# gonewest818/raytrace-clj

Hardware: NVIDIA B200
Metric: samples_per_sec (higher is better)
Workload: dtype f32

## Files before the change

### raytrace_clj_b200/csrc/rt_kernels.cuh

```cuda
#pragma once

#include "rt_device.cuh"

namespace rt {

#define RT_FOR_R _Pragma("unroll") for (int r = 0; r < R; ++r)

struct PathBounce {
    float o[3];
    float time;
    float d[3];
    int hit_id;
    double t;
};

struct RenderParams {
    DevScene sc;
    DevCamera cam;
    int nx, ny;
    int sample_begin, sample_count;
    int row_offset, row_stride, rows_in_shard;
    int max_depth;
    uint2 key;
    float* sum;
// ... 440 lines not shown
    }
}

template <int R, int BLOCK>
struct PairSink {
    unsigned idx0;
    unsigned n;
    unsigned n_g, p0;
    __device__ __forceinline__ unsigned entry(unsigned v) const { return v < n_g ? v : p0 + (v - n_g); }
    unsigned long long live;
    uint2* pairs;
    unsigned pair_cap;
    unsigned long long* best_key;
    WaveState* st;

    __device__ __forceinline__ void flush(const uint32_t* list, unsigned long long nz, int count, int kbase) {
        nz &= live;
        if (!__any_sync(0xffffffffu, nz != 0ull)) return;
        const unsigned lane = threadIdx.x & 31u;
        unsigned np = 0;
        for (unsigned long long z = nz; z; z &= z - 1ull) {
            const int i = __ffsll((long long)z) - 1;
            np += __popc(~Culler<R, BLOCK>::word(list, i & 15, i >> 4));
        }
        unsigned incl = np;
#pragma unroll
        for (int d = 1; d < 32; d <<= 1) {
            unsigned v = __shfl_up_sync(0xffffffffu, incl, d);
            if ((int)lane >= d) incl += v;
        }
        const unsigned total = __shfl_sync(0xffffffffu, incl, 31);
        unsigned base = 0;
        if (lane == 0) base = atomicAdd(&st->npairs, total);
        base = __shfl_sync(0xffffffffu, base, 0);
        const bool fits = base + total <= pair_cap;
        unsigned w = base + incl - np;
        SurvivorIter<R, BLOCK> it;
        it.begin(nz, count);
        int r, k;
        while (it.next(list, r, k)) {
            const unsigned v = idx0 + 32u * (unsigned)r;
            if (fits) {
                pairs[w] = make_uint2(entry(v), (unsigned)(kbase + k));
            } else {
                if (w < pair_cap) pairs[w] = make_uint2(PAIR_NULL, 0u);
                if (v < n) best_key[entry(v)] = BEST_KEY_OVERFLOW;
            }
            ++w;
        }
    }
};

constexpr unsigned ITEM_NONE = 0xffffffffu;
constexpr unsigned ITEM_STOP = 0xfffffffeu;
struct Scope {
    unsigned bid, nblk;
};
__device__ __forceinline__ Scope grid_scope() { return Scope{blockIdx.x, gridDim.x}; }
template <int R, int BLOCK, bool COMMON>
__device__ __forceinline__ unsigned wf_cull_batches(const WaveParams& W, Scope sc_, int cur, unsigned e0, unsigned e1, unsigned n_g,
                                                    unsigned p0, unsigned long long gen0, int parts, unsigned item0, unsigned claimed,
                                                    int& budget, float4* s_cull, uint32_t* s_list) {
    if (claimed == ITEM_STOP) return ITEM_STOP;
    const RenderParams& P = W.base;
    const unsigned lane = threadIdx.x & 31u, warp = threadIdx.x >> 5, warps = BLOCK / 32;
    const unsigned n_batches = (e1 - e0 + 32 * R - 1) / (32 * R);
    const unsigned n_items = n_batches * (unsigned)parts;
    Culler<R, BLOCK, COMMON> K;
    K.cox = P.cam.origin.x; K.coy = P.cam.origin.y; K.coz = P.cam.origin.z;
    PairSink<R, BLOCK> sink;
    sink.n = e1;
    sink.n_g = n_g;
    sink.p0 = p0;
    sink.pairs = W.pairs;
    sink.pair_cap = W.pair_cap;
    sink.best_key = W.best_key;
    sink.st = W.st;
    unsigned item = sc_.bid * warps + warp;
    const unsigned uniform_end = (n_items + warps - 1) / warps * warps;
    for (;;) {
        if (P.preloaded) {
            if (claimed != ITEM_NONE) {
                item = claimed;
                claimed = ITEM_NONE;
            } else {
                unsigned b = 0;
                if (lane == 0) b = atomicAdd(&W.st->batch, 1u);
                item = __shfl_sync(0xffffffffu, b, 0);
            }
            if (item >= item0 + n_items) return item;
            item -= item0;
        } else {
            if (item - warp >= uniform_end) break;
        }
        const unsigned batch = item / (unsigned)parts, part = item - batch * (unsigned)parts;
        sink.idx0 = e0 + batch * (32 * R) + lane;
        sink.live = 0ull;
        RT_FOR_R {
            const unsigned v = sink.idx0 + 32 * r;
            if (v < e1 && batch < n_batches) {
                float4* qc = cur ? W.queue[1] : W.queue[0];
                float4 a, b;
                if (v >= n_g) {
                    float4 c;
                    float4* q = qc + 3 * (size_t)(p0 + (v - n_g));
                    make_path(P, gen0 + (v - n_g), a, b, c);
                    if (part == 0) { q[0] = a; q[1] = b; q[2] = c; }
                } else {
                    a = qc[3 * (size_t)v];
                    b = qc[3 * (size_t)v + 1];
                }
                K.set_ray(r, a.x, a.y, a.z, b.x, b.y, b.z);
                sink.live |= 0xffffull << (16 * r);
            } else {
                K.kill(r);
            }
        }
        if (parts > 1) K.run_slice(P.sc, s_cull, s_list, sink, (int)part, parts);
        else           K.run(P.sc, s_cull, P.cull_cap, P.preloaded != 0, s_list, sink);
        item += sc_.nblk * warps;
        if (P.preloaded && budget > 0 && --budget == 0) return ITEM_STOP;
    }
    return ITEM_NONE;
}

template <int R, int BLOCK>
__device__ __forceinline__ void wf_cull_body(const WaveParams& W, Scope sc_, int cur, unsigned n_g, unsigned n_p, unsigned long long gen_base,
                                             float4* s_cull, float4* s_cullc, uint32_t* s_list) {
    const RenderParams& P = W.base;
    const unsigned n = n_g + n_p, p0 = (unsigned)W.capacity - n_p;
    if (sc_.bid == 0 && threadIdx.x == 0) atomicAdd(&P.counters[DC_RAYS], (unsigned long long)n);
    const unsigned grid_warps = W.resident_warps > 0 ? (unsigned)W.resident_warps : sc_.nblk * (BLOCK / 32);
    int budget = W.claims_per_warp;
    const unsigned n_c = P.common_origin ? n_p : 0u, n_v = n - n_c;
    const unsigned long long genC = gen_base - p0;
    if (R > 1 && !P.preloaded) {
        if (n_c) wf_cull_batches<R, BLOCK, true>(W, sc_, cur, p0, p0 + n_c, 0u, 0u, genC + 0u, 1, 0u, ITEM_NONE, budget, s_cull, s_list);
        if (n_v) wf_cull_batches<R, BLOCK, false>(W, sc_, cur, 0u, n_v, n_g, p0, gen_base, 1, 0u, ITEM_NONE, budget, s_cull, s_list);
    } else if (R > 1 && n >= grid_warps * 64u) {
        const unsigned tail = grid_warps * 64u, per = 32u * R;
        const unsigned g_rest0 = min(n_v, tail), p_rest0 = min(n_c, tail - g_rest0);
        const unsigned g_bulk = (n_v - g_rest0) / per * per, p_bulk = (n_c - p_rest0) / per * per;
        unsigned items = 0;
        unsigned next = wf_cull_batches<R, BLOCK, true>(W, sc_, cur, p0, p0 + p_bulk, 0u, 0u, genC, 1, items, ITEM_NONE, budget, s_cullc, s_list);
        items += p_bulk / per;
        next = wf_cull_batches<R, BLOCK, false>(W, sc_, cur, 0u, g_bulk, n_g, p0, gen_base, 1, items, next, budget, s_cull, s_list);
        items += g_bulk / per;
        next = wf_cull_batches<1, BLOCK, true>(W, sc_, cur, p0 + p_bulk, p0 + n_c, 0u, 0u, genC, 1, items, next, budget, s_cullc, s_list);
        items += (n_c - p_bulk + 31u) / 32u;
        wf_cull_batches<1, BLOCK, false>(W, sc_, cur, g_bulk, n_v, n_g, p0, gen_base, 1, items, next, budget, s_cull, s_list);
    } else {
        const unsigned b1 = (n + 31) / 32;
        int parts = 1;
        if (P.preloaded)
            while (parts < 16 && b1 * (unsigned)parts * 2u <= grid_warps) parts *= 2;
        unsigned next = ITEM_NONE, items = 0;
        if (n_c) {
            next = wf_cull_batches<1, BLOCK, true>(W, sc_, cur, p0, p0 + n_c, 0u, 0u, genC, parts, 0u, ITEM_NONE, budget, P.preloaded ? s_cullc : s_cull, s_list);
            items = (n_c + 31u) / 32u * (unsigned)parts;
        }
        if (n_v) wf_cull_batches<1, BLOCK, false>(W, sc_, cur, 0u, n_v, n_g, p0, gen_base, parts, items, next, budget, s_cull, s_list);
    }
}

template <int R, int BLOCK, int MINB>
__global__ void __launch_bounds__(BLOCK, MINB) wf_cull(const __grid_constant__ WaveParams W) {
    TraceScope trace(W.trace);
    const RenderParams& P = W.base;
    extern __shared__ float4 smem_f4[];
    float4* s_cull = smem_f4;
    uint32_t* s_list = reinterpret_cast<uint32_t*>(smem_f4 + P.cull_cap);
    float4* s_cullc = reinterpret_cast<float4*>(s_list + Culler<R, BLOCK>::LIST_WORDS * BLOCK);
    if (W.st->mode != MODE_RUN) return;
    const unsigned n_g = W.st->cnt[W.cur][0], n_p = W.st->cnt[W.cur][1];
    if (n_g + n_p == 0) return;
    const unsigned long long gen_base = W.st->gen_base[W.cur];
    if (P.preloaded) {
        preload_scene(P.sc, s_cull, BLOCK);
        if (n_p && P.common_origin)
            for (int i = threadIdx.x; i < P.sc.n_cull; i += BLOCK)
                s_cullc[i] = Culler<R, BLOCK, true>::common_record(s_cull[i], P.cam.origin.x, P.cam.origin.y, P.cam.origin.z);
    }
    __syncthreads();
    wf_cull_body<R, BLOCK>(W, grid_scope(), W.cur, n_g, n_p, gen_base, s_cull, s_cullc, s_list);
}

#include "rt_cull_tc.cuh"

__device__ __forceinline__ unsigned wf_cand_region(const WaveParams& W, unsigned total_warps) {
    return ((W.pair_cap + total_warps * 32u - 1u) / (total_warps * 32u)) * 32u;
}

template <bool GEN>
__device__ __forceinline__ void wf_refine_body(const WaveParams& W, const DevScene* scp, Scope sc_, int cur) {
    const RenderParams& P = W.base;
    const unsigned npairs = min(W.st->npairs, W.pair_cap);
    const unsigned lane = threadIdx.x & 31u;
    if (sc_.bid == 0 && threadIdx.x == 0) {
        W.st->batch = 0;
        W.st->cnt[cur ^ 1][0] = 0;
        W.st->cnt[cur ^ 1][1] = 0;
        atomicAdd(&P.counters[DC_CANDIDATES], (unsigned long long)(npairs - min(npairs, W.st->pad)));
        W.st->pad = 0;
    }
    const unsigned total_warps = sc_.nblk * (blockDim.x >> 5);
    const unsigned warp_id = sc_.bid * (blockDim.x >> 5) + (threadIdx.x >> 5);
    const size_t region = (size_t)warp_id * wf_cand_region(W, total_warps);
    unsigned cnt = 0;
    const unsigned stride = sc_.nblk * blockDim.x;
    const unsigned i_first = sc_.bid * blockDim.x + threadIdx.x;
    uint2 pr_next = i_first < npairs ? W.pairs[i_first] : make_uint2(PAIR_NULL, 0u);
    for (unsigned i0 = i_first - lane; i0 < npairs; i0 += stride) {
        const uint2 pr = pr_next;
        const unsigned i_next = i0 + lane + stride;
        pr_next = i_next < npairs ? W.pairs[i_next] : make_uint2(PAIR_NULL, 0u);
        bool cand = false;
        double t = CUDART_INF;
        if (pr.x != PAIR_NULL) {
            const float4* qc = cur ? W.queue[1] : W.queue[0];
            const float4 a = qc[3 * (size_t)pr.x], b = qc[3 * (size_t)pr.x + 1];
            const unsigned long long seen = __ldcg(&W.best_t[pr.x]);
            if (!GEN) {
                t = refine_candidate(P.sc.ex_c0r, P.sc.ex_c1, P.sc.ex_t0t1, P.sc.flags, (int)pr.y, a.x, a.y, a.z, b.x, b.y, b.z,
                                     a.w, 0.001, (double)FLT_MAX);
            } else {
                uint32_t pixq = 0, smpq = 0, bq = 0;
                if (__ldg(&P.sc.prim_type[pr.y]) == PRIM_MEDIUM) {
                    const uint32_t sd = __float_as_uint(qc[3 * (size_t)pr.x + 2].w);
                    pixq = rng_pixel(P, __float_as_uint(b.w));
                    smpq = sd >> 8;
                    bq = (uint32_t)(P.max_depth - (int)(sd & 255u) + 1);
                }
                t = refine_leaf<true>(scp, (int)pr.y, a.x, a.y, a.z, b.x, b.y, b.z, a.w, 0.001, (double)FLT_MAX, true, P.key, pixq, smpq, bq);
            }
            const unsigned long long tb = (unsigned long long)__double_as_longlong(t);
            if (t < CUDART_INF && tb <= seen) {
                atomicMin(&W.best_t[pr.x], tb);
                cand = true;
            }
        }
        const unsigned m = __ballot_sync(0xffffffffu, cand);
        if (cand) {
            const size_t slot = region + cnt + __popc(m & ((1u << lane) - 1u));
            W.cands[slot] = pr;
            W.cand_t[slot] = t;
        }
        cnt += __popc(m);
    }
    if (lane == 0) W.cand_count[warp_id] = cnt;
}
template <bool GEN>
__global__ void __launch_bounds__(256) wf_refine(const __grid_constant__ WaveParams W) {
    if (W.st->mode != MODE_RUN) return;
    TraceScope trace(W.trace);
    wf_refine_body<GEN>(W, &W.base.sc, grid_scope(), W.cur);
}

__device__ __forceinline__ void wf_tiebreak_body(const WaveParams& W, Scope sc_) {
    const RenderParams& P = W.base;
    const unsigned lane = threadIdx.x & 31u;
    const unsigned total_warps = sc_.nblk * (blockDim.x >> 5);
    const unsigned warp_id = sc_.bid * (blockDim.x >> 5) + (threadIdx.x >> 5);
    const size_t region = (size_t)warp_id * wf_cand_region(W, total_warps);
    const unsigned cnt = W.cand_count[warp_id];
    for (unsigned j = lane; j < cnt; j += 32) {
        const uint2 pr = W.cands[region + j];
        if ((unsigned long long)__double_as_longlong(W.cand_t[region + j]) == W.best_t[pr.x])
            atomicMin(&W.best_key[pr.x], (((unsigned long long)__ldg(&P.sc.tie_hi[pr.y])) << 32) | pr.y);
    }
}
__global__ void __launch_bounds__(256) wf_tiebreak(const __grid_constant__ WaveParams W) {
    if (W.st->mode != MODE_RUN) return;
    TraceScope trace(W.trace);
    wf_tiebreak_body(W, grid_scope());
}

template <bool GEN>
__device__ __noinline__ void exact_closest_hit(const DevScene* sc, float ox, float oy, float oz, float dx, float dy, float dz,
                                               float tm, uint2 key, uint32_t pixel, uint32_t sample, uint32_t bounce, double* out_t,
                                               int* out_k) {
    double best = CUDART_INF;
    int bk = -1;
    unsigned btie = 0xffffffffu;
    for (int k = 0; k < sc->n; ++k) {
        double t = refine_leaf<GEN>(sc, k, ox, oy, oz, dx, dy, dz, tm, 0.001, (double)FLT_MAX, true, key, pixel, sample, bounce);
        if (t < CUDART_INF) {
            unsigned tie = __ldg(&sc->tie_hi[k]);
            if (t < best || (t == best && tie < btie)) { best = t; bk = k; btie = tie; }
        }
    }
    *out_t = best;
    *out_k = bk;
}

template <bool GEN>
__device__ __forceinline__ unsigned wf_shade_body(const WaveParams& W, const DevScene* scp, Scope sc_, int cur, unsigned* s_ctr) {
    const RenderParams& P = W.base;
    const unsigned n_g = W.st->cnt[cur][0], n_p = W.st->cnt[cur][1], n = n_g + n_p;
    const unsigned lane = threadIdx.x & 31u;
    const float4* qc = cur ? W.queue[1] : W.queue[0];
    float4* qn = cur ? W.queue[0] : W.queue[1];
    if (sc_.bid == 0 && threadIdx.x == 0) W.st->npairs = 0;
    unsigned n_direct = 0;
    const unsigned stride = sc_.nblk * blockDim.x;
    for (unsigned idx0 = sc_.bid * blockDim.x + threadIdx.x - lane; idx0 < n; idx0 += stride) {
        const bool have = idx0 + lane < n;
        const unsigned idx = wf_entry(idx0 + lane, n_g, n_p, (unsigned)W.capacity);
        bool cont = false;
        float4 a, b, c;
        if (have) {
            a = qc[3 * (size_t)idx]; b = qc[3 * (size_t)idx + 1]; c = qc[3 * (size_t)idx + 2];
            unsigned long long key = W.best_key[idx];
            const uint32_t slot = __float_as_uint(b.w), sd = __float_as_uint(c.w);
            const uint32_t pix = rng_pixel(P, slot);
            const uint32_t smp = sd >> 8;
            const int depth = (int)(sd & 255u);
            const uint32_t bounce = (uint32_t)(P.max_depth - depth + 1);
            int k = (int)(unsigned)key;
            double td = __longlong_as_double((long long)W.best_t[idx]);
            W.best_key[idx] = BEST_KEY_MISS;
            W.best_t[idx] = BEST_T_INIT;
            if (key == BEST_KEY_OVERFLOW) {
                exact_closest_hit<GEN>(scp, a.x, a.y, a.z, b.x, b.y, b.z, a.w, P.key, pix, smp, bounce, &td, &k);
                key = k < 0 ? BEST_KEY_MISS : 1ull;
            } else {
                for (int kd = P.sc.n_list; kd < P.sc.n; ++kd) {
                    ++n_direct;
                    const double t = refine_leaf<GEN>(scp, kd, a.x, a.y, a.z, b.x, b.y, b.z, a.w, 0.001, (double)FLT_MAX, true, P.key, pix,
                                                      smp, bounce);
                    const unsigned long long kk = (((unsigned long long)__ldg(&P.sc.tie_hi[kd])) << 32) | (unsigned)kd;
                    if (t < td || (t < CUDART_INF && t == td && kk < key)) {
                        td = t;
                        key = kk;
                        k = kd;
                    }
                }
            }
            const bool hit = key != BEST_KEY_MISS;
            if (P.path_pixel) path_log_ray(P, slot, (int)bounce - 1, a, b, hit ? k : -1, hit ? td : CUDART_INF);
            if (!hit) {
                atomicAdd(&s_ctr[DC_TERM_MISS], 1u);
                if (P.path_pixel) path_log_end(P, slot, (int)bounce, TERM_MISS);
            } else {
                float3 o = f3(a.x, a.y, a.z), d = f3(b.x, b.y, b.z);
                float3 att, em;
                int reason = TERM_NONE;
                float tmv = a.w;
                ScatterRng rng{P.key, pix, smp, bounce, nullptr, nullptr};
                cont = shade_hit<GEN>(P.sc, scp, k, (float)td, o, d, tmv, depth > 0, rng, att, em, reason);
                if (em.x != 0.f || em.y != 0.f || em.z != 0.f) {
                    float* dst = P.sum + (size_t)slot * 3;
                    atomicAdd(dst + 0, c.x * em.x);
                    atomicAdd(dst + 1, c.y * em.y);
                    atomicAdd(dst + 2, c.z * em.z);
                }
                if (cont) {
                    a = make_float4(o.x, o.y, o.z, tmv);
                    b = make_float4(d.x, d.y, d.z, b.w);
                    c = make_float4(c.x * att.x, c.y * att.y, c.z * att.z, __uint_as_float((smp << 8) | (uint32_t)(depth - 1)));
                } else {
                    atomicAdd(&s_ctr[reason == TERM_LIGHT ? DC_TERM_LIGHT
                                     : reason == TERM_ABSORB ? DC_TERM_ABSORB : DC_TERM_DEPTH], 1u);
                    if (P.path_pixel) path_log_end(P, slot, (int)bounce, reason);
                }
            }
        }
        const unsigned mc = __ballot_sync(0xffffffffu, cont);
        if (mc) {
            unsigned base = 0u;
            if (lane == 0) base = atomicAdd(&W.st->cnt[cur ^ 1][0], (unsigned)__popc(mc));
            base = __shfl_sync(0xffffffffu, base, 0);
            if (cont) {
                float4* q = qn + 3 * (size_t)(base + __popc(mc & ((1u << lane) - 1u)));
                q[0] = a; q[1] = b; q[2] = c;
            }
        }
    }
    if (n_direct) atomicAdd(&s_ctr[DC_DIRECT], n_direct);
    return 0u;
}

template <bool GEN>
__global__ void __launch_bounds__(256, GEN ? 1 : 0) wf_shade(const __grid_constant__ WaveParams W) {
    if (W.st->mode != MODE_RUN) return;
    TraceScope trace(W.trace);
    const RenderParams& P = W.base;
    __shared__ unsigned s_ctr[DC_COUNT];
    if (threadIdx.x < DC_COUNT) s_ctr[threadIdx.x] = 0;
    __syncthreads();
    wf_shade_body<GEN>(W, &W.base.sc, grid_scope(), W.cur, s_ctr);
    __syncthreads();
    if (threadIdx.x < DC_COUNT && s_ctr[threadIdx.x]) atomicAdd(&P.counters[threadIdx.x], (unsigned long long)s_ctr[threadIdx.x]);
    if (threadIdx.x == 0) {
        __threadfence();
        if (atomicAdd(&W.st->done, 1u) == gridDim.x - 1) {
            __threadfence();
            W.st->done = 0;
            const unsigned n_cont = *(volatile unsigned*)&W.st->cnt[W.cur ^ 1][0];
            const unsigned want = (unsigned)W.capacity - n_cont;
            unsigned n_fresh = 0;
            unsigned long long base = 0ull;
            if (!W.st->exhausted && want) {
                base = atomicAdd(P.work_counter, (unsigned long long)want);
                if (base < P.total_work) n_fresh = (unsigned)min((unsigned long long)want, P.total_work - base);
                if (base + want >= P.total_work) W.st->exhausted = 1u;
            }
            W.st->cnt[W.cur ^ 1][1] = n_fresh;
            W.st->gen_base[W.cur ^ 1] = base;
            if (n_fresh) atomicAdd(&P.counters[DC_SAMPLES], (unsigned long long)n_fresh);
            if (n_cont + n_fresh == 0) W.st->mode = MODE_DONE;
            __threadfence();
            publish_status(W, n_cont + n_fresh, n_fresh, W.st->exhausted, W.st->mode, W.iter);
        }
    }
}

struct TraceParamsB {
    DevScene sc;
    int n;
    const float* origins;
    const float* dirs;
    const float* times;
    double tmin, tmax;
    double* out_t;
    int* out_id;
    unsigned long long* stats;
};

struct BvhHit {
    double t;
    int k;
    unsigned tie;
    unsigned n_leaf, n_node;
};
template <bool GEN>
__device__ __forceinline__ BvhHit bvh_closest(const DevScene* sc, float ox, float oy, float oz, float dx, float dy, float dz, float time,
                                              double tmin, double tmax, bool has_ctx, uint2 key, uint32_t pixel, uint32_t sample,
                                              uint32_t bounce) {
    BvhHit H{CUDART_INF, -1, 0xffffffffu, 0u, 0u};
    const float ix = 1.0f / dx, iy = 1.0f / dy, iz = 1.0f / dz;
    const float e = 2.4e-7f * fmaxf(fmaxf(fabsf(ox), fabsf(oy)), fabsf(oz));
    const float tlo = (float)tmin * (1.0f - 1e-6f);
    float thi = tmax >= (double)FLT_MAX ? FLT_MAX : __double2float_ru(tmax);
    int stack[48];
    int sp = 0, node = 0;
    for (;;) {
        if (node >= 0) {
            const float4 A = __ldg(&sc->bvh[4 * node]), B = __ldg(&sc->bvh[4 * node + 1]), C = __ldg(&sc->bvh[4 * node + 2]);
            const int4 D = __ldg(reinterpret_cast<const int4*>(&sc->bvh[4 * node + 3]));
            H.n_node += 2;
            float a0 = ((A.x - e) - ox) * ix, a1 = ((A.w + e) - ox) * ix, b0 = ((A.y - e) - oy) * iy, b1 = ((B.x + e) - oy) * iy,
                  c0 = ((A.z - e) - oz) * iz, c1 = ((B.y + e) - oz) * iz;
            float ln = fmaxf(fmaxf(fminf(a0, a1), fminf(b0, b1)), fmaxf(fminf(c0, c1), tlo));
            float lf = fminf(fminf(fmaxf(a0, a1), fmaxf(b0, b1)), fminf(fmaxf(c0, c1), thi));
            a0 = ((B.z - e) - ox) * ix; a1 = ((C.y + e) - ox) * ix; b0 = ((B.w - e) - oy) * iy; b1 = ((C.z + e) - oy) * iy;
            c0 = ((C.x - e) - oz) * iz; c1 = ((C.w + e) - oz) * iz;
            float rn = fmaxf(fmaxf(fminf(a0, a1), fminf(b0, b1)), fmaxf(fminf(c0, c1), tlo));
            float rf = fminf(fminf(fmaxf(a0, a1), fmaxf(b0, b1)), fminf(fmaxf(c0, c1), thi));
            const bool hl = ln <= lf * 1.0000005f + 1e-30f, hr = rn <= rf * 1.0000005f + 1e-30f;
            if (hl && hr) {
                const bool left_first = ln <= rn;
                stack[sp++] = left_first ? D.y : D.x;
                node = left_first ? D.x : D.y;
                continue;
            }
            if (hl) { node = D.x; continue; }
            if (hr) { node = D.y; continue; }
        } else {
            const int k = ~node;
            H.n_leaf++;
            const double t = refine_leaf<GEN>(sc, k, ox, oy, oz, dx, dy, dz, time, tmin, tmax, has_ctx, key, pixel, sample, bounce);
            if (t < CUDART_INF) {
                const unsigned tie = __ldg(&sc->tie_hi[k]);
                if (t < H.t || (t == H.t && tie < H.tie)) {
                    H.t = t; H.k = k; H.tie = tie;
                    thi = fminf(thi, __double2float_ru(t));
                }
            }
        }
        if (sp == 0) break;
        node = stack[--sp];
    }
    return H;
}

template <bool GEN>
__global__ void __launch_bounds__(128, GEN ? 1 : 0) wf_bvh(const __grid_constant__ WaveParams W) {
    if (W.st->mode != MODE_RUN) return;
    TraceScope trace(W.trace);
    const RenderParams& P = W.base;
    __shared__ unsigned s_ctr[DC_COUNT];
    if (threadIdx.x < DC_COUNT) s_ctr[threadIdx.x] = 0;
    __syncthreads();
    const int cur = W.cur;
    const unsigned n_g = W.st->cnt[cur][0], n_p = W.st->cnt[cur][1], n = n_g + n_p, p0 = (unsigned)W.capacity - n_p;
    const unsigned long long gen_base = W.st->gen_base[cur];
    float4* qc = cur ? W.queue[1] : W.queue[0];
    unsigned n_leaf = 0, n_node = 0;
    for (unsigned v = blockIdx.x * blockDim.x + threadIdx.x; v < n; v += gridDim.x * blockDim.x) {
        float4 a, b, c;
        unsigned idx;
        if (v >= n_g) {
            idx = p0 + (v - n_g);
            make_path(P, gen_base + (v - n_g), a, b, c);
            float4* q = qc + 3 * (size_t)idx;
            q[0] = a; q[1] = b; q[2] = c;
        } else {
            idx = v;
            a = qc[3 * (size_t)idx]; b = qc[3 * (size_t)idx + 1]; c = qc[3 * (size_t)idx + 2];
        }
        const uint32_t sd = __float_as_uint(c.w);
        const BvhHit H = bvh_closest<GEN>(&W.base.sc, a.x, a.y, a.z, b.x, b.y, b.z, a.w, 0.001, (double)FLT_MAX, true, P.key,
                                          rng_pixel(P, __float_as_uint(b.w)), sd >> 8, (uint32_t)(P.max_depth - (int)(sd & 255u) + 1));
        n_leaf += H.n_leaf; n_node += H.n_node;
        if (H.k >= 0) {
            W.best_t[idx] = (unsigned long long)__double_as_longlong(H.t);
            W.best_key[idx] = ((unsigned long long)H.tie << 32) | (unsigned)H.k;
        }
    }
    atomicAdd(&s_ctr[DC_CANDIDATES], n_leaf);
    atomicAdd(&s_ctr[DC_BVH_NODES], n_node);
    __syncthreads();
    if (threadIdx.x < DC_COUNT && s_ctr[threadIdx.x]) atomicAdd(&P.counters[threadIdx.x], (unsigned long long)s_ctr[threadIdx.x]);
    if (blockIdx.x == 0 && threadIdx.x == 0) {
        atomicAdd(&P.counters[DC_RAYS], (unsigned long long)n);
        W.st->batch = 0;
        W.st->npairs = 0;
        W.st->cnt[cur ^ 1][0] = 0;
        W.st->cnt[cur ^ 1][1] = 0;
    }
}

template <bool GEN>
__global__ void __launch_bounds__(128) trace_bvh_kernel(const __grid_constant__ TraceParamsB P) {
    const int idx = blockIdx.x * blockDim.x + threadIdx.x;
    if (idx >= P.n) return;
    const float ox = P.origins[3 * idx], oy = P.origins[3 * idx + 1], oz = P.origins[3 * idx + 2];
    const float dx = P.dirs[3 * idx], dy = P.dirs[3 * idx + 1], dz = P.dirs[3 * idx + 2];
    const float tm = P.times ? P.times[idx] : 0.f;
    BvhHit H = bvh_closest<GEN>(&P.sc, ox, oy, oz, dx, dy, dz, tm, P.tmin, P.tmax, false, make_uint2(0u, 0u), 0u, 0u, 0u);
    for (int k = P.sc.n_list; k < P.sc.n; ++k) {
        const double t = refine_leaf<GEN>(&P.sc, k, ox, oy, oz, dx, dy, dz, tm, P.tmin, P.tmax, false, make_uint2(0u, 0u), 0u, 0u, 0u);
        const unsigned tie = __ldg(&P.sc.tie_hi[k]);
        if (t < H.t || (t < CUDART_INF && t == H.t && tie < H.tie)) { H.t = t; H.k = k; H.tie = tie; }
    }
    P.out_t[idx] = H.t;
    P.out_id[idx] = H.k >= 0 ? __ldg(&P.sc.orig_id[H.k]) : -1;
    if (P.stats) {
        atomicAdd(&P.stats[0], (unsigned long long)H.n_leaf);
        atomicAdd(&P.stats[1], (unsigned long long)H.n_node);
    }
}

template <bool GEN>
__device__ __forceinline__ void wf_solo_paths(const WaveParams& W, const DevScene* scp, const float4* qc, unsigned n, unsigned* claim,
                                              const float4* s_cull, unsigned* s_ctr) {
    const RenderParams& P = W.base;
    const unsigned lane = threadIdx.x & 31u;
    const unsigned lpp = W.tail_lpp;
    const unsigned sub = lane & (lpp - 1u), lead = lane & ~(lpp - 1u);
    bool active = false;
    float4 a = make_float4(0.f, 0.f, 0.f, 0.f), b = a, c = a;
    uint32_t slot = 0u, pix = 0u;
    unsigned n_rays = 0, n_cand = 0, n_direct = 0;
    for (;;) {
        unsigned i = 0xffffffffu;
        if (!active && sub == 0u) i = atomicAdd(claim, 1u);
        i = __shfl_sync(0xffffffffu, i, (int)lead);
        if (!active && i < n) {
            a = qc[3 * (size_t)i]; b = qc[3 * (size_t)i + 1]; c = qc[3 * (size_t)i + 2];
            slot = __float_as_uint(b.w);
            pix = rng_pixel(P, slot);
            active = true;
        }
        if (!__any_sync(0xffffffffu, active)) break;
        const uint32_t sd = __float_as_uint(c.w), smp = sd >> 8;
        const int depth = (int)(sd & 255u);
        const uint32_t bounce = (uint32_t)(P.max_depth - depth + 1);
        Culler<1, 32, false> K;
        K.set_ray(0, a.x, a.y, a.z, b.x, b.y, b.z);
        if (active && sub == 0u) ++n_rays;
        unsigned long long bt = BEST_T_INIT, bkey = BEST_KEY_MISS;
        for (int base = 0; base < P.sc.n; base += 64 * (int)lpp) {
            unsigned long long mask = 0ull;
            if (active) {
                const int jn = min(64, (P.sc.n - base + (int)lpp - 1) / (int)lpp);
#pragma unroll 4
                for (int j = 0; j < jn; ++j) {
                    const int s = base + (int)lpp * j + (int)sub;
                    bool pass = s < P.sc.n;
                    if (s < P.sc.n_list) {
                        const float4 S = P.preloaded ? s_cull[s] : __ldg(&P.sc.cull_a[s]);
                        pass = (int)K.key_bits(S, 0) >= 0;
                    }
                    mask |= (unsigned long long)(pass ? 1u : 0u) << j;
                }
            }
            while (__any_sync(0xffffffffu, mask != 0ull)) {
                if (mask) {
                    const int s = base + (int)lpp * (__ffsll((long long)mask) - 1) + (int)sub;
                    mask &= mask - 1ull;
                    if (s < P.sc.n_list) ++n_cand; else ++n_direct;
                    const double t = refine_leaf<GEN>(scp, s, a.x, a.y, a.z, b.x, b.y, b.z, a.w, 0.001, (double)FLT_MAX, true, P.key, pix, smp,
                                                      bounce);
                    const unsigned long long tb = (unsigned long long)__double_as_longlong(t);
                    const unsigned long long kk = (((unsigned long long)__ldg(&P.sc.tie_hi[s])) << 32) | (unsigned)s;
                    if (t < CUDART_INF && (tb < bt || (tb == bt && kk < bkey))) { bt = tb; bkey = kk; }
                }
            }
        }
        for (unsigned dlt = lpp >> 1; dlt; dlt >>= 1) {
            const unsigned long long ot = __shfl_xor_sync(0xffffffffu, bt, (int)dlt), ok = __shfl_xor_sync(0xffffffffu, bkey, (int)dlt);
            if (ot < bt || (ot == bt && ok < bkey)) { bt = ot; bkey = ok; }
        }
        if (active) {
            const bool hit = bkey != BEST_KEY_MISS;
            const int k = (int)(unsigned)bkey;
            const double td = __longlong_as_double((long long)bt);
            if (P.path_pixel && sub == 0u) path_log_ray(P, slot, (int)bounce - 1, a, b, hit ? k : -1, hit ? td : CUDART_INF);
            int reason = TERM_MISS;
            bool cont = false;
            if (hit) {
                float3 o = f3(a.x, a.y, a.z), d = f3(b.x, b.y, b.z);
                float3 att, em;
                float tmv = a.w;
                ScatterRng rng{P.key, pix, smp, bounce, nullptr, nullptr};
                reason = TERM_NONE;
                cont = shade_hit<GEN>(P.sc, scp, k, (float)td, o, d, tmv, depth > 0, rng, att, em, reason);
                if (sub == 0u && (em.x != 0.f || em.y != 0.f || em.z != 0.f)) {
                    float* dst = P.sum + (size_t)slot * 3;
                    atomicAdd(dst + 0, c.x * em.x);
                    atomicAdd(dst + 1, c.y * em.y);
                    atomicAdd(dst + 2, c.z * em.z);
                }
                if (cont) {
                    a = make_float4(o.x, o.y, o.z, tmv);
                    b = make_float4(d.x, d.y, d.z, b.w);
                    c = make_float4(c.x * att.x, c.y * att.y, c.z * att.z, __uint_as_float((smp << 8) | (uint32_t)(depth - 1)));
                }
            }
            if (!cont) {
                if (sub == 0u) {
                    atomicAdd(&s_ctr[reason == TERM_MISS ? DC_TERM_MISS : reason == TERM_LIGHT ? DC_TERM_LIGHT
                                     : reason == TERM_ABSORB ? DC_TERM_ABSORB : DC_TERM_DEPTH], 1u);
                    if (P.path_pixel) path_log_end(P, slot, (int)bounce, reason);
                }
                active = false;
            }
        }
    }
    if (n_rays) atomicAdd(&s_ctr[DC_RAYS], n_rays);
    if (n_cand) atomicAdd(&s_ctr[DC_CANDIDATES], n_cand);
    if (n_direct) atomicAdd(&s_ctr[DC_DIRECT], n_direct);
}

constexpr int kPairsPerEntry = 8;
template <int BLOCK, bool GEN, int TR>
__global__ void __launch_bounds__(BLOCK, GEN ? 1 : 2) wf_tail(const __grid_constant__ WaveParams W) {
    const RenderParams& P = W.base;
    extern __shared__ float4 smem_f4[];
    float4* s_cull = smem_f4;
    uint32_t* s_list = reinterpret_cast<uint32_t*>(smem_f4 + P.cull_cap);
    __shared__ unsigned s_ctr[DC_COUNT];
    __shared__ WaveState s_st;
    if (W.st->mode == MODE_DONE) return;
    TraceScope trace(W.trace);
    int cur = W.cur;
    const unsigned n_all = W.st->cnt[cur][0];
    const unsigned K = ((n_all + gridDim.x - 1) / gridDim.x + 31u) / 32u * 32u;
    const unsigned first = blockIdx.x * K;
    if (first < n_all) {
        if (threadIdx.x < DC_COUNT) s_ctr[threadIdx.x] = 0;
        if (threadIdx.x == 0) {
            s_st.cnt[cur][0] = min(K, n_all - first);
            s_st.cnt[cur ^ 1][0] = 0;
            s_st.cnt[0][1] = s_st.cnt[1][1] = 0;
            s_st.gen_base[0] = s_st.gen_base[1] = 0ull;
            s_st.batch = 0;
// ... 432 lines not shown
```

Before: 1.618 billion.

## Prefetch next queue entry and aggregate continuation-queue appends per block

The shade loop now loads the next iteration's ray origin, direction, best key and best t in software-pipelined fashion, so those global loads overlap with shading of the current entry. The per-warp atomicAdd on the next-queue counter is replaced by a block-level prefix over warp counts in shared memory with a single atomic per block iteration. This reduces global atomic contention and hides load latency, but adds two __syncthreads per iteration. It also assumes at most 8 warps per block and that all threads in the block run the same number of loop iterations, which holds because the loop bound is block-uniform.

```diff
diff --git a/raytrace_clj_b200/csrc/rt_kernels.cuh b/raytrace_clj_b200/csrc/rt_kernels.cuh
--- a/raytrace_clj_b200/csrc/rt_kernels.cuh
+++ b/raytrace_clj_b200/csrc/rt_kernels.cuh
@@ -766,22 +766,34 @@
     float4* qn = cur ? W.queue[0] : W.queue[1];
     if (sc_.bid == 0 && threadIdx.x == 0) W.st->npairs = 0;
     unsigned n_direct = 0;
-    const unsigned stride = sc_.nblk * blockDim.x;
-    for (unsigned idx0 = sc_.bid * blockDim.x + threadIdx.x - lane; idx0 < n; idx0 += stride) {
-        const bool have = idx0 + lane < n;
-        const unsigned idx = wf_entry(idx0 + lane, n_g, n_p, (unsigned)W.capacity);
+    const unsigned stride = sc_.nblk * blockDim.x, warp = threadIdx.x >> 5;
+    __shared__ unsigned s_warp_cnt[8], s_warp_off[8];
+    unsigned idx_next = 0u;
+    float4 a_next, b_next;
+    unsigned long long key_next = 0ull, t_next = 0ull;
+    auto load_entry = [&](unsigned v) {
+        idx_next = wf_entry(min(v, n - 1u), n_g, n_p, (unsigned)W.capacity);
+        a_next = qc[3 * (size_t)idx_next]; b_next = qc[3 * (size_t)idx_next + 1];
+        key_next = W.best_key[idx_next];
+        t_next = W.best_t[idx_next];
+    };
+    if (n) load_entry(sc_.bid * blockDim.x + threadIdx.x);
+    for (unsigned base0 = sc_.bid * blockDim.x; base0 < n; base0 += stride) {
+        const bool have = base0 + threadIdx.x < n;
+        const unsigned idx = idx_next;
+        float4 a = a_next, b = b_next, c;
+        unsigned long long key = key_next;
+        const unsigned long long t_bits = t_next;
+        if (have) c = qc[3 * (size_t)idx + 2];
         bool cont = false;
-        float4 a, b, c;
         if (have) {
-            a = qc[3 * (size_t)idx]; b = qc[3 * (size_t)idx + 1]; c = qc[3 * (size_t)idx + 2];
-            unsigned long long key = W.best_key[idx];
             const uint32_t slot = __float_as_uint(b.w), sd = __float_as_uint(c.w);
             const uint32_t pix = rng_pixel(P, slot);
             const uint32_t smp = sd >> 8;
             const int depth = (int)(sd & 255u);
             const uint32_t bounce = (uint32_t)(P.max_depth - depth + 1);
             int k = (int)(unsigned)key;
-            double td = __longlong_as_double((long long)W.best_t[idx]);
+            double td = __longlong_as_double((long long)t_bits);
             W.best_key[idx] = BEST_KEY_MISS;
             W.best_t[idx] = BEST_T_INIT;
             if (key == BEST_KEY_OVERFLOW) {
@@ -828,16 +840,25 @@
                     if (P.path_pixel) path_log_end(P, slot, (int)bounce, reason);
                 }
             }
+            load_entry(base0 + stride + threadIdx.x);
         }
         const unsigned mc = __ballot_sync(0xffffffffu, cont);
-        if (mc) {
-            unsigned base = 0u;
-            if (lane == 0) base = atomicAdd(&W.st->cnt[cur ^ 1][0], (unsigned)__popc(mc));
-            base = __shfl_sync(0xffffffffu, base, 0);
-            if (cont) {
-                float4* q = qn + 3 * (size_t)(base + __popc(mc & ((1u << lane) - 1u)));
-                q[0] = a; q[1] = b; q[2] = c;
-            }
+        if (lane == 0) s_warp_cnt[warp] = __popc(mc);
+        __syncthreads();
+        if (threadIdx.x == 0) {
+            unsigned total = 0u;
+            for (unsigned w = 0; w < (blockDim.x >> 5); ++w) {
+                const unsigned c_w = s_warp_cnt[w];
+                s_warp_off[w] = total;
+                total += c_w;
+            }
+            const unsigned base = total ? atomicAdd(&W.st->cnt[cur ^ 1][0], total) : 0u;
+            for (unsigned w = 0; w < (blockDim.x >> 5); ++w) s_warp_off[w] += base;
+        }
+        __syncthreads();
+        if (cont) {
+            float4* q = qn + 3 * (size_t)(s_warp_off[warp] + __popc(mc & ((1u << lane) - 1u)));
+            q[0] = a; q[1] = b; q[2] = c;
         }
     }
     if (n_direct) atomicAdd(&s_ctr[DC_DIRECT], n_direct);
```

New measurement: 1.683 billion (median of 6 runs). 4.0% higher.
